# NingZhang1/pyscf_isdf

Measured on AMD Instinct MI355X. Metric: isdf_build_plus_get_jk_wall_time, lower is better.
Workload: dtype f64

## Files before the change

### include/mi355_isdf.h

```cpp
#ifndef MI355_ISDF_H
#define MI355_ISDF_H

#include <stdint.h>

#ifdef __cplusplus
extern "C" {
#endif

typedef struct isdf_ctx* isdf_handle;

#define ISDF_OK 0
#define ISDF_ERR_ARG 1
#define ISDF_ERR_HIP 2
#define ISDF_ERR_LIB 3
#define ISDF_ERR_NUM 4

int isdf_abi_version(void);

int isdf_create(int device_id, isdf_handle* out);
int isdf_destroy(isdf_handle h);
int isdf_set_stream(isdf_handle h, void* hip_stream);
const char* isdf_last_error(isdf_handle h);
int64_t isdf_workspace_bytes(isdf_handle h);
int isdf_release_workspace(isdf_handle h);
// ... 24 lines not shown
                          const double* d_coords, int64_t ngrids, double* d_re, double* d_im, int64_t ld,
                          int64_t plane_stride);

int isdf_eval_ao_k(isdf_handle h,
                   const int32_t* atm, int natm, const int32_t* bas, int nbas,
                   const double* env, int nenv,
                   const double* Ls, int nimgs, const double* rcut,
                   const double kpt[3], int periodic_part,
                   const double* d_coords, int64_t ngrids,
                   double* d_re, double* d_im, int64_t ld);

int isdf_block_row_absmax(isdf_handle h, const double* d_src, int nrow, int64_t ld, int nblk, const int64_t* d_blk_off,
                          double* d_out);
int isdf_gather_cols(isdf_handle h, const double* d_src, int nrow, int64_t ld_src,
                     const int64_t* d_idx, int64_t n, double* d_dst, int64_t ld_dst);

int isdf_partition_by_atom(isdf_handle h, const double* d_coords, int64_t ngrids, const double* atom_coords, int natm,
                           const double a[9], double tie_atol, int32_t* d_owner);

int isdf_select_ip(isdf_handle h, const double* d_ao, int nao, int64_t ld,
                   int nblk, const int64_t* blk_off, const int32_t* nip,
                   double tol, double tie_rtol,
                   double* d_L, int64_t ldL, int64_t* d_piv, int32_t* rank);

int isdf_select_ip_ws(isdf_handle h, const double* d_ao, int nao, int64_t ld,
                      int nblk, const int64_t* blk_off, const int32_t* nip,
                      double tol, double tie_rtol,
                      double* d_L, int64_t ldL, int64_t* d_piv, int32_t* rank,
                      void* d_work, int64_t work_bytes);
int64_t isdf_select_ip_work_bytes(int nao, int64_t m);

int isdf_select_ip_gram(isdf_handle h, double* d_A, int m, int64_t ldA, int nip, double tol, double tie_rtol,
                        int panel, int64_t* d_piv, int32_t* rank);

int isdf_select_ip_cplx(isdf_handle h, const double* d_ao, int nao, int nh, int64_t ld,
                        int nblk, const int64_t* blk_off, const int32_t* nip,
                        double tol, double tie_rtol,
                        double* d_L, int64_t ldL, int64_t* d_piv, int32_t* rank);

int isdf_fit_from_chol(isdf_handle h, double* d_L, int k, int64_t m, int64_t ldL,
                       const int64_t* d_piv);

int isdf_fit_prepare(isdf_handle h, const double* d_ao, int nao, int64_t ld,
                     const int64_t* d_ip, int P, double reg_rel, double* d_aoP, double* d_chol,
                     double* reg_used);
int isdf_fit_apply(isdf_handle h, const double* d_chol, const double* d_aoP, int P, int nao,
                   const double* d_ao, int64_t ng, int64_t ld, int forward_only,
                   double* d_theta, int64_t ldt);
int isdf_fit_prepare_cplx(isdf_handle h, const double* d_ao, int nao, int nh, int64_t ld,
                          const int64_t* d_ip, int P, double reg_rel, double* d_aoP, double* d_chol,
                          double* reg_used);
int isdf_fit_apply_cplx(isdf_handle h, const double* d_chol, const double* d_aoP, int P, int nao, int nh,
                        const double* d_ao, int64_t ng, int64_t ld, int forward_only,
                        double* d_theta, int64_t ldt);
int isdf_fit_global(isdf_handle h, const double* d_ao, int nao, int64_t ngrids, int64_t ld,
                    const int64_t* d_ip, int P, double reg_rel, double* d_theta, int64_t ldt,
                    double* d_aoP, double* reg_used);

int isdf_gather_aoP(isdf_handle h, const double* d_ao, int nao, int64_t ld, const int64_t* d_ip, int P,
                    double* d_aoP);
int isdf_gram_sq(isdf_handle h, const double* d_aoP, int P, int nao, int nh, double* d_A);
int isdf_pair_gram_rows(isdf_handle h, const double* d_aoP, int P, int nao, int nh, const double* d_ao,
                        int64_t ng, int64_t ld, double* d_B, int64_t ldb);
int isdf_block_chol(isdf_handle h, const double* d_A, int P, int nblk, const int32_t* blk_off,
                    double shift_rel, double* d_D, double* shift_used);
int isdf_block_solve(isdf_handle h, const double* d_D, int P, int nblk, const int32_t* blk_off, int side,
// ... 144 lines not shown
```

### pyscf_isdf_amd/backend.py

```python
import ctypes
import os
import numpy as np
import torch
from . import lib as _lib

_vp = ctypes.c_void_p


def _np_ptr(a):
    return a.ctypes.data_as(_vp)


class HipBackend:
    name = 'hip-gfx950'

    def __init__(self, device=0):
        if not torch.cuda.is_available():
            raise _lib.IsdfError('no GPU visible to torch; the ISDF path has no CPU fallback')
        self.device = torch.device('cuda', device)
        torch.cuda.set_device(self.device)
        self.handle = _lib.Handle(device)
        if os.environ.get('ISDF_TRSM') == 'subst':
            self.set_option('trsm_substitution', 1)
        if os.environ.get('ISDF_OWN_FFT') in ('0', '1', '2'):
# ... 157 lines not shown
        self._stream()
        coords_soa = self.to_device(np.ascontiguousarray(np.asarray(coords, dtype=np.float64).T))
        atoms = np.ascontiguousarray(atom_coords, dtype=np.float64)
        a = np.ascontiguousarray(a, dtype=np.float64)
        G = coords_soa.shape[1]
        owner = self.empty((G,), dtype=torch.int32)
        self.handle.call('isdf_partition_by_atom', self._p(coords_soa), G, _np_ptr(atoms), len(atoms), _np_ptr(a), float(tie_atol),
                         self._p(owner))
        return self.to_host(owner)

    def select_ip_work_bytes(self, nao, m):
        return int(self.handle.lib.isdf_select_ip_work_bytes(int(nao), int(m)))

    def select_ip(self, ao, blk_off, nip, tol, tie_rtol, L, piv, work=None):
        self._stream()
        blk_off = np.ascontiguousarray(blk_off, dtype=np.int64)
        nip = np.ascontiguousarray(nip, dtype=np.int32)
        rank = np.zeros(len(nip), dtype=np.int32)
        assert piv.dtype == torch.int64 and piv.is_contiguous() and ao.stride(1) == 1 and L.stride(1) == 1
        assert work is None or work.is_contiguous()
        self.handle.call('isdf_select_ip_ws', self._p(ao), ao.shape[0], ao.stride(0), len(nip), _np_ptr(blk_off),
                         _np_ptr(nip), float(tol), float(tie_rtol), self._p(L), L.stride(0), self._p(piv), _np_ptr(rank),
                         None if work is None else self._p(work), 0 if work is None else work.numel() * work.element_size())
        return rank

    def select_ip_gram(self, A, nip, tol, tie_rtol, piv, panel=0):
        self._stream()
        assert piv.dtype == torch.int64 and piv.is_contiguous() and A.stride(1) == 1 and A.shape[0] == A.shape[1]
        rank = ctypes.c_int32(0)
        self.handle.call('isdf_select_ip_gram', self._p(A), A.shape[0], A.stride(0), int(nip), float(tol), float(tie_rtol),
                         int(panel), self._p(piv), ctypes.byref(rank))
        return int(rank.value)

    def fit_from_chol(self, L, k, m, piv):
        self._stream()
        self.handle.call('isdf_fit_from_chol', self._p(L), int(k), int(m), L.stride(0), self._p(piv))

    def fit_prepare(self, ao, ip, reg_rel, aoP, chol):
        self._stream()
        assert ip.dtype == torch.int64 and aoP.is_contiguous() and chol.is_contiguous()
        reg = ctypes.c_double(0.0)
        self.handle.call('isdf_fit_prepare', self._p(ao), ao.shape[0], ao.stride(0), self._p(ip), ip.numel(),
                         float(reg_rel), self._p(aoP), self._p(chol), ctypes.byref(reg))
        return reg.value

    def fit_apply(self, chol, aoP, ao, ng, theta, forward_only=False):
        self._stream()
        self.handle.call('isdf_fit_apply', self._p(chol), self._p(aoP), aoP.shape[0], aoP.shape[1], self._p(ao),
                         int(ng), ao.stride(0), int(bool(forward_only)), self._p(theta), theta.stride(0))

    def gather_aoP(self, ao, ip, aoP):
        self._stream()
        self.handle.call('isdf_gather_aoP', self._p(ao), ao.shape[0], ao.stride(0), self._p(ip), ip.numel(), self._p(aoP))

    def gram_sq(self, aoP, A, nh=0):
        self._stream()
        self.handle.call('isdf_gram_sq', self._p(aoP), aoP.shape[0], aoP.shape[1], int(nh), self._p(A))

    def pair_gram_rows(self, aoP, ao, ng, B, nh=0):
        self._stream()
        self.handle.call('isdf_pair_gram_rows', self._p(aoP), aoP.shape[0], aoP.shape[1], int(nh), self._p(ao), int(ng),
                         ao.stride(0), self._p(B), B.stride(0))

    def gram_prod(self, aoP, psiP, A):
        self._stream()
        assert aoP.is_contiguous() and psiP.is_contiguous() and A.is_contiguous() and aoP.shape[0] == psiP.shape[0]
# ... 476 lines not shown
```

### pyscf_isdf_amd/csrc/common.h

```cpp
#pragma once
#include <hip/hip_runtime.h>
#include <rocblas/rocblas.h>
#include <rocsolver/rocsolver.h>
#include <hipfft/hipfft.h>
#include <cstdint>
#include <cstdio>
#include <cstring>
#include <string>
#include <vector>
#include <map>
#include "../../include/mi355_isdf.h"

struct FftPlan {
  hipfftHandle fwd = 0, bwd = 0;
  size_t work_bytes = 0;
};

struct ProfRec {
  hipEvent_t e0 = nullptr, e1 = nullptr;
};
struct ProfEntry {
  std::vector<ProfRec> recs;
  double work = 0.0;
  double ms = 0.0;
  int64_t launches = 0;
};

struct WsKernel {
  double alpha = 0.0;
  double ak[9] = {0};
  int mesh[3] = {0, 0, 0};
  double maxq[3] = {0, 0, 0};
  const double* vq = nullptr;
};

struct isdf_ctx {
  int profiling = 0;
  std::map<std::string, ProfEntry> prof;
  int device = 0;
  hipStream_t stream = nullptr;
  rocblas_handle blas = nullptr;
  std::string err;
  std::map<std::vector<int>, FftPlan> plans;
  std::map<std::string, std::pair<void*, size_t>> ws;
  int num_cu = 256;
  int trsm_substitution = 0;
  int own_fft = 2;
  int gemm_nn_own = 0;
  int attr_gemm_b = 0, attr_gemm_nn = 0, attr_gram_tri = 0, attr_herm = 0;
  int cand_gram = 1;
  int conv_pipe = 1;
  int conv_sub_rows = 0;
  int gram_pivot_tpb = 256;
  int gram_compact = 1;
  int gram_compact_permille = 875;
  int block_apply_waves = 16;
  int block_apply_reg = 1;
  double coul_omega = 0.0;
  double coul_rc = 0.0;
  int coul_sphere = 0;
  WsKernel wsk;
};

int isdf_fail(isdf_handle h, int code, const char* fmt, ...);
void* isdf_ws(isdf_handle h, const char* name, size_t bytes);
int isdf_get_plan(isdf_handle h, const int32_t mesh[3], int batch, FftPlan** out);
int get_coulG_half(isdf_handle h, const int32_t mesh[3], const double a[9], double extra_scale, double** out);
bool conv_rows_own_supported(const int32_t mesh[3], int nb);
bool conv_rows_q_own_supported(isdf_handle h, const int32_t mesh[3], int nb);
bool spectral_rows_own_supported(isdf_handle h, const int32_t mesh[3], int nb);
int spectral_rows_own(isdf_handle h, const double* d_in, int nb, const int32_t mesh[3], const int32_t* d_idx, const double* d_scale,
                      int npts, double* d_out, int64_t ldx, HIP_vector_type<double, 2u>* zbuf);
int conv_rows_q_own(isdf_handle h, const double* d_in, double* d_re, double* d_im, int nb, const int32_t mesh[3], const double* tab,
                    double2* zhalf, double2* zfull);
int conv_rows_own(isdf_handle h, const double* d_in, double* d_out, int nb, const int32_t mesh[3], const double* cg,
                  double2* zbuf);

#define HIP_TRY(h, expr)                                                                    \
  do {                                                                                      \
    hipError_t e_ = (expr);                                                                 \
    if (e_ != hipSuccess)                                                                   \
      return isdf_fail(h, ISDF_ERR_HIP, "%s:%d %s -> %s", __FILE__, __LINE__, #expr,        \
                       hipGetErrorString(e_));                                              \
  } while (0)
#define BLAS_TRY(h, expr)                                                                   \
  do {                                                                                      \
    rocblas_status s_ = (expr);                                                             \
    if (s_ != rocblas_status_success)                                                       \
// ... 35 lines not shown
  }
};

int gemm_nt_f64(isdf_handle h, int M, int N, int64_t K, double alpha, const double* A, int64_t lda,
                const double* B, int64_t ldb, double beta, double* C, int64_t ldc);
int gemm_nt_f64_scaled(isdf_handle h, int M, int N, int64_t K, double alpha, const double* A, int64_t lda,
                       const double* B, int64_t ldb, const double* kscale, double beta, double* C,
                       int64_t ldc);
int trsm_lower_left(isdf_handle h, bool trans, int m, int64_t n, const double* L, int64_t ldl, double* X, int64_t ldx);
int trsm_lower_right(isdf_handle h, bool trans, int m, int64_t n, const double* L, int64_t ldl, double* X, int64_t ldx);
int block_forward_solve(isdf_handle h, const double* D, int64_t ldd, int nblk, const int32_t* blk_off_host, double* X,
                        int64_t ldx, int64_t n);
int block_apply_inverse(isdf_handle h, const double* Dinv, int64_t ldd, int nblk, const int32_t* blk_off_host, double* X,
                        int64_t ldx, int64_t n, bool square_input = false);
int transpose_rm(isdf_handle h, const double* src, int64_t lds, int64_t rows, int64_t cols, double* dst, int64_t ldd);
int tri_left(isdf_handle h, bool trans, int m, int64_t n, const double* L, int64_t ldl, double* X, int64_t ldx);
int tri_right(isdf_handle h, bool trans, int m, int64_t n, const double* L, int64_t ldl, double* X, int64_t ldx);
bool gemm_nn_f64_supported(isdf_handle h, int64_t M, int64_t N, int64_t K, const double* A, int64_t lda, const double* B,
                           int64_t ldb);
int gemm_nn_f64(isdf_handle h, int64_t M, int64_t N, int64_t K, const double* A, int64_t lda, const double* B, int64_t ldb,
                double* C, int64_t ldc, bool square);
int gemm_rm(isdf_handle h, char opA, char opB, int64_t M, int64_t N, int64_t K, double alpha,
            const double* A, int64_t lda, const double* B, int64_t ldb, double beta, double* C,
            int64_t ldc);

__host__ __device__ inline int64_t gram_tri_row(int64_t r) {
  const int64_t tm = r >> 8;
  return 32768 * tm * (tm + 1) + (r & 255) * ((tm + 1) << 8);
}
static inline int64_t gram_tri_size(int64_t m) { return m > 0 ? gram_tri_row(m - 1) + (((m - 1) >> 8) + 1) * 256 : 0; }
struct GramTriUnit { int blk, tm, tn, pad; };
int gram_tri_blocks(isdf_handle h, const double* X, int64_t ldx, int K, const GramTriUnit* d_units, int64_t nunits,
                    const int64_t* d_blk_off, int64_t row0, const int64_t* d_tri_off, double* S, double flop);
```

### pyscf_isdf_amd/csrc/gemm_f64.hip

```cpp
#include "common.h"
#include <cstdlib>

int gemm_rm(isdf_handle h, char opA, char opB, int64_t M, int64_t N, int64_t K, double alpha,
            const double* A, int64_t lda, const double* B, int64_t ldb, double beta, double* C,
            int64_t ldc) {
  ARG_CHECK(h, M < 2147483647LL && N < 2147483647LL && K < 2147483647LL && lda < 2147483647LL &&
                   ldb < 2147483647LL && ldc < 2147483647LL);
  const rocblas_operation ta = (opA == 'N') ? rocblas_operation_none : rocblas_operation_transpose;
  const rocblas_operation tb = (opB == 'N') ? rocblas_operation_none : rocblas_operation_transpose;
  ProfScope ps(h, "rocblas_dgemm[flop]", 2.0 * M * N * (double)K);
  BLAS_TRY(h, rocblas_dgemm(h->blas, tb, ta, (rocblas_int)N, (rocblas_int)M, (rocblas_int)K, &alpha, B,
                            (rocblas_int)ldb, A, (rocblas_int)lda, &beta, C, (rocblas_int)ldc));
  return ISDF_OK;
}

namespace {

typedef double d4 __attribute__((ext_vector_type(4)));

constexpr int BM = 128, BN = 128, BK = 16;
constexpr int LDT = 17;
constexpr int TPB = 256;

struct GemmArgs {
// ... 148 lines not shown
struct GramTriArgs {
  const double* X; int64_t ldx; int K;
  const GramTriUnit* units;
  const int64_t* blk_off;
  int64_t row0;
  const int64_t* tri_off;
  double* S;
  int64_t nunits, nunits_pad;
};

__global__ __launch_bounds__(TPB2, 2) void gram_tri_mfma_kernel(GramTriArgs t) {
  extern __shared__ double smem[];
  const int64_t bid = blockIdx.x;
  const int64_t per_xcd = t.nunits_pad / 8;
  const int64_t unit = (bid % 8) * per_xcd + bid / 8;
  if (unit >= t.nunits) return;
  const GramTriUnit u = t.units[unit];
  const int64_t r0 = t.blk_off[u.blk];
  GemmArgs g;
  g.A = g.B = t.X + (r0 - t.row0) * t.ldx;
  g.lda = g.ldb = t.ldx;
  g.kscale = nullptr;
  g.M = g.N = (int)(t.blk_off[u.blk + 1] - r0);
  g.K = g.kslab = t.K;
  g.ldp = (int64_t)(u.tm + 1) * BM2;
  g.P = t.S + t.tri_off[u.blk] + (gram_tri_row((int64_t)u.tm * BM2) - (int64_t)u.tm * BM2 * g.ldp);
  g.slab_stride = 0;
  g.direct = 1; g.alpha = 1.0; g.beta = 0.0;
  constexpr bool SCALED = false;
  double* sA = smem;
  double* sB = smem + 2 * BM2 * LDT;
  const int tm = u.tm, tn = u.tn, slab = 0;
#include "gemm_nt_b_unit.inc"
}

constexpr int TPBD = 256;

template <bool SCALED>
__global__ __launch_bounds__(TPBD, 2) void gemm_nt_mfma_kernel_d(GemmArgs g) {
  __shared__ double sB[2][BN * LDT];
  const int64_t bid = blockIdx.x;
  const int64_t per_xcd = g.nunits_pad / 8;
  const int64_t unit = (bid % 8) * per_xcd + bid / 8;
  if (unit >= g.nunits) return;
  const int tm = (int)(unit % g.ntm);
  const int tn = (int)((unit / g.ntm) % g.ntn);
  const int slab = (int)(unit / ((int64_t)g.ntm * g.ntn));
  const int64_t k0 = (int64_t)slab * g.kslab;
  const int64_t k1 = (k0 + g.kslab < g.K) ? k0 + g.kslab : g.K;
  const int nchunks = (int)((k1 - k0) / BK);
  const int last = nchunks - 1;

  const int tid = threadIdx.x;
  const int lane = tid & 63, wave = tid >> 6;
  const int frow = lane & 15, fkq = lane >> 4;
  const int mlast = g.M - 1, nlast = g.N - 1;
  const double* pA0 = g.A + (int64_t)min(tm * BM + wave * 32 + frow, mlast) * g.lda + k0 + 4 * fkq;
  const double* pA1 = g.A + (int64_t)min(tm * BM + wave * 32 + 16 + frow, mlast) * g.lda + k0 + 4 * fkq;
  const int srow = tid >> 2, sseg = tid & 3;
  const double* pB0 = g.B + (int64_t)min(tn * BN + srow, nlast) * g.ldb + k0 + 4 * sseg;
  const double* pB1 = g.B + (int64_t)min(tn * BN + srow + 64, nlast) * g.ldb + k0 + 4 * sseg;
  const double* pS = SCALED ? g.kscale + k0 + 4 * sseg : nullptr;

  double2 xa00, xa01, xa10, xa11, xb00, xb01, xb10, xb11;
  double2 ya00, ya01, ya10, ya11, yb00, yb01, yb10, yb11;
#define ISDF_LOADD(C, A00, A01, A10, A11, B00, B01, B10, B11)                                 \
// ... 540 lines not shown
}

int gemm_nt_f64(isdf_handle h, int M, int N, int64_t K, double alpha, const double* A, int64_t lda,
                const double* B, int64_t ldb, double beta, double* C, int64_t ldc) {
  return gemm_nt_f64_scaled(h, M, N, K, alpha, A, lda, B, ldb, nullptr, beta, C, ldc);
}

extern "C" int isdf_gemm_nt(isdf_handle h, int M, int N, int64_t K, double alpha, const double* d_A,
                            int64_t lda, const double* d_B, int64_t ldb, const double* d_kscale,
                            double beta, double* d_C, int64_t ldc) {
  if (!h) return ISDF_ERR_ARG;
  return gemm_nt_f64_scaled(h, M, N, K, alpha, d_A, lda, d_B, ldb, d_kscale, beta, d_C, ldc);
}

int gram_tri_blocks(isdf_handle h, const double* X, int64_t ldx, int K, const GramTriUnit* d_units, int64_t nunits,
                    const int64_t* d_blk_off, int64_t row0, const int64_t* d_tri_off, double* S, double flop) {
  ARG_CHECK(h, X && d_units && d_blk_off && d_tri_off && S && nunits > 0 && K > 0 && K % 32 == 0 && ldx >= K && ldx % 2 == 0 &&
                   ((uintptr_t)X) % 16 == 0);
  GramTriArgs t;
  t.X = X; t.ldx = ldx; t.K = K; t.units = d_units; t.blk_off = d_blk_off; t.row0 = row0; t.tri_off = d_tri_off; t.S = S;
  t.nunits = nunits; t.nunits_pad = cdiv(nunits, 8) * 8;
  ARG_CHECK(h, t.nunits_pad < 2147483647LL);
  const size_t lds = sizeof(double) * 2 * (BM2 + BN) * LDT;
  if (!h->attr_gram_tri) {
    HIP_TRY(h, hipFuncSetAttribute((const void*)gram_tri_mfma_kernel, hipFuncAttributeMaxDynamicSharedMemorySize, (int)lds));
    h->attr_gram_tri = 1;
  }
  ProfScope ps(h, "cand_gram_blocks[flop]", flop);
  hipLaunchKernelGGL(gram_tri_mfma_kernel, dim3((unsigned)t.nunits_pad), dim3(TPB2), lds, h->stream, t);
  KERNEL_CHECK(h);
  return ISDF_OK;
}

bool gemm_nn_f64_supported(isdf_handle h, int64_t M, int64_t N, int64_t K, const double* A, int64_t lda, const double* B,
                           int64_t ldb) {
  return h->gemm_nn_own && M > BM && (double)(cdiv(M, BM2) * BM2) <= 1.15 * (double)M && N >= 2 && N % 2 == 0 && K >= 32 && K % 32 == 0 &&
         lda % 2 == 0 && ldb % 2 == 0 && ((uintptr_t)A) % 16 == 0 && ((uintptr_t)B) % 16 == 0 && M < 2147483647LL &&
         N < 2147483647LL && K < 2147483647LL;
}

int gemm_nn_f64(isdf_handle h, int64_t M, int64_t N, int64_t K, const double* A, int64_t lda, const double* B, int64_t ldb,
                double* C, int64_t ldc, bool square) {
  ARG_CHECK(h, A && B && C && lda >= K && ldb >= N && ldc >= N && gemm_nn_f64_supported(h, M, N, K, A, lda, B, ldb));
  GemmNNArgs g;
  g.A = A; g.lda = lda; g.B = B; g.ldb = ldb; g.C = C; g.ldc = ldc;
  g.M = (int)M; g.N = (int)N; g.K = (int)K;
  g.ntm = (int)cdiv(M, BM2); g.ntn = (int)cdiv(N, BN);
  g.stm = g.ntm >= 4 ? 4 : (g.ntm >= 2 ? 2 : 1);
  g.stn = 32 / g.stm;
  g.ngm = (int)cdiv(g.ntm, g.stm);
  g.nunits = (int64_t)g.ngm * cdiv(g.ntn, g.stn) * 32;
  g.nunits_pad = cdiv(g.nunits, 8) * 8;
  ARG_CHECK(h, g.nunits_pad < 2147483647LL);
  const size_t lds = sizeof(double) * 2 * (BM2 * LDT + BK * LDN);
  if (!h->attr_gemm_nn) {
    HIP_TRY(h, hipFuncSetAttribute((const void*)gemm_nn_mfma_kernel<true>, hipFuncAttributeMaxDynamicSharedMemorySize, (int)lds));
    HIP_TRY(h, hipFuncSetAttribute((const void*)gemm_nn_mfma_kernel<false>, hipFuncAttributeMaxDynamicSharedMemorySize, (int)lds));
    h->attr_gemm_nn = 1;
  }
  ProfScope ps(h, square ? "gemm_nn_mfma_kernel<true>[flop]" : "gemm_nn_mfma_kernel<false>[flop]", 2.0 * M * N * (double)K);
  if (square) hipLaunchKernelGGL(gemm_nn_mfma_kernel<true>, dim3((unsigned)g.nunits_pad), dim3(TPB2), lds, h->stream, g);
  else hipLaunchKernelGGL(gemm_nn_mfma_kernel<false>, dim3((unsigned)g.nunits_pad), dim3(TPB2), lds, h->stream, g);
  KERNEL_CHECK(h);
  return ISDF_OK;
}
```

### pyscf_isdf_amd/csrc/gemm_nt_b_unit.inc

```
  const int64_t k0 = (int64_t)slab * g.kslab;
  const int64_t k1 = (k0 + g.kslab < g.K) ? k0 + g.kslab : g.K;
  const int nchunks = (int)((k1 - k0) / BK);
  const int last = nchunks - 1;

  const int tid = threadIdx.x;
  const int lane = tid & 63, wave = tid >> 6;
  const int wm = wave >> 1, wn = wave & 1;
  const int srow = tid >> 3;
  const int sseg = tid & 7;
  const int mlast = g.M - 1, nlast = g.N - 1;
  const double* pA0 = g.A + (int64_t)min(tm * BM2 + srow, mlast) * g.lda + k0 + sseg * 2;
  const double* pA1 = g.A + (int64_t)min(tm * BM2 + srow + 64, mlast) * g.lda + k0 + sseg * 2;
  const double* pA2 = g.A + (int64_t)min(tm * BM2 + srow + 128, mlast) * g.lda + k0 + sseg * 2;
  const double* pA3 = g.A + (int64_t)min(tm * BM2 + srow + 192, mlast) * g.lda + k0 + sseg * 2;
  const double* pB0 = g.B + (int64_t)min(tn * BN + srow, nlast) * g.ldb + k0 + sseg * 2;
  const double* pB1 = g.B + (int64_t)min(tn * BN + srow + 64, nlast) * g.ldb + k0 + sseg * 2;
  const double* pS = SCALED ? g.kscale + k0 + sseg * 2 : nullptr;

  double2 xa0, xa1, xa2, xa3, xb0, xb1, ya0, ya1, ya2, ya3, yb0, yb1;
#define ISDF_LOADB(C, A0, A1, A2, A3, B0, B1)                                                 \
  {                                                                                           \
    const int off = (C) * BK;                                                                 \
    A0 = *reinterpret_cast<const double2*>(pA0 + off);                                        \
    A1 = *reinterpret_cast<const double2*>(pA1 + off);                                        \
// ... 56 lines not shown
  {                                                                                           \
    ISDF_FRAGQ(BUF, 1, a1, b1)                                                                \
    LOAD_AHEAD                                                                                \
    ISDF_MFMAB(a0, b0)                                                                        \
    ISDF_INTERLEAVE_L()                                                                       \
    __builtin_amdgcn_sched_barrier(0);                                                        \
    ISDF_FRAGQ(BUF, 2, a0, b0)                                                                \
    ISDF_MFMAB(a1, b1)                                                                        \
    ISDF_INTERLEAVE()                                                                         \
    __builtin_amdgcn_sched_barrier(0);                                                        \
    ISDF_FRAGQ(BUF, 3, a1, b1)                                                                \
    STORE_NEXT                                                                                \
    ISDF_MFMAB(a0, b0)                                                                        \
    ISDF_INTERLEAVE_RW()                                                                      \
    __builtin_amdgcn_sched_barrier(0);                                                        \
    __syncthreads();                                                                          \
    ISDF_FRAGQ(1 - (BUF), 0, a0, b0)                                                          \
    ISDF_MFMAB(a1, b1)                                                                        \
    ISDF_INTERLEAVE()                                                                         \
    __builtin_amdgcn_sched_barrier(0);                                                        \
  }

  ISDF_LOADB(0, xa0, xa1, xa2, xa3, xb0, xb1)
  ISDF_LOADB(1, ya0, ya1, ya2, ya3, yb0, yb1)
  ISDF_STOREB(0, xa0, xa1, xa2, xa3, xb0, xb1)
  __syncthreads();
  ISDF_FRAGQ(0, 0, a0, b0)
  __builtin_amdgcn_sched_barrier(0);
  for (int c = 0; c < nchunks; c += 2) {
    ISDF_CHUNKB(0, ISDF_LOADB(min(c + 2, last), xa0, xa1, xa2, xa3, xb0, xb1), ISDF_STOREB(1, ya0, ya1, ya2, ya3, yb0, yb1))
    ISDF_CHUNKB(1, ISDF_LOADB(min(c + 3, last), ya0, ya1, ya2, ya3, yb0, yb1), ISDF_STOREB(0, xa0, xa1, xa2, xa3, xb0, xb1))
  }

  double* out = g.P + (int64_t)slab * g.slab_stride;
#pragma unroll
  for (int i = 0; i < 4; ++i) {
#pragma unroll
    for (int r = 0; r < 4; ++r) {
      const int row = tm * BM2 + wm * 64 + i * 16 + (lane >> 4) + 4 * r;
      if (row >= g.M) continue;
#pragma unroll
      for (int j = 0; j < 4; ++j) {
        const int col = tn * BN + wn * 64 + j * 16 + (lane & 15);
        if (col >= g.N) continue;
        double* q = out + (int64_t)row * g.ldp + col;
        const double v = acc[i][j][r];
        if (g.direct) *q = (g.beta == 0.0) ? g.alpha * v : g.alpha * v + g.beta * (*q);
        else *q = v;
      }
    }
  }
```

### pyscf_isdf_amd/csrc/handle.hip

```cpp
#include "common.h"
#include <cstdarg>

int isdf_fail(isdf_handle h, int code, const char* fmt, ...) {
  char buf[1024];
  va_list ap;
  va_start(ap, fmt);
  vsnprintf(buf, sizeof(buf), fmt, ap);
  va_end(ap);
  if (h) h->err = buf;
  else fprintf(stderr, "mi355_isdf: %s\n", buf);
  return code;
}

void* isdf_ws(isdf_handle h, const char* name, size_t bytes) {
  auto& slot = h->ws[name];
  if (slot.second >= bytes && slot.first) return slot.first;
  if (slot.first) {
    (void)hipStreamSynchronize(h->stream);
    (void)hipFree(slot.first);
    slot.first = nullptr;
    slot.second = 0;
  }
  void* p = nullptr;
  hipError_t e = hipMalloc(&p, bytes ? bytes : 8);
// ... 49 lines not shown
  ARG_CHECK(h, rc >= 0.0);
  h->coul_rc = rc;
  return ISDF_OK;
}

int isdf_set_coulomb_ws(isdf_handle h, double alpha, const double ak[9], const int32_t mesh[3], const double maxq[3],
                        const double* d_vq) {
  if (!h) return ISDF_ERR_ARG;
  if (alpha <= 0.0) { h->wsk = WsKernel(); return ISDF_OK; }
  ARG_CHECK(h, ak && mesh && maxq && d_vq && mesh[0] > 0 && mesh[1] > 0 && mesh[2] > 0);
  h->wsk.alpha = alpha;
  for (int i = 0; i < 9; ++i) h->wsk.ak[i] = ak[i];
  for (int i = 0; i < 3; ++i) { h->wsk.mesh[i] = mesh[i]; h->wsk.maxq[i] = maxq[i]; }
  h->wsk.vq = d_vq;
  return ISDF_OK;
}

int isdf_set_option(isdf_handle h, const char* key, int value) {
  if (!h) return ISDF_ERR_ARG;
  ARG_CHECK(h, key != nullptr);
  if (std::string(key) == "trsm_substitution") { h->trsm_substitution = value ? 1 : 0; return ISDF_OK; }
  if (std::string(key) == "own_fft") { h->own_fft = value < 0 ? 0 : (value > 2 ? 2 : value); return ISDF_OK; }
  if (std::string(key) == "gemm_nn_own") { h->gemm_nn_own = value ? 1 : 0; return ISDF_OK; }
  if (std::string(key) == "coul_sphere") { h->coul_sphere = value < 0 ? 0 : value; return ISDF_OK; }
  if (std::string(key) == "conv_pipe") { h->conv_pipe = value != 0; return ISDF_OK; }
  if (std::string(key) == "conv_sub_rows") { h->conv_sub_rows = value < 0 ? 0 : value; return ISDF_OK; }
  if (std::string(key) == "gram_pivot_tpb") {
    if (value != 64 && value != 128 && value != 256) return ISDF_ERR_ARG;
    h->gram_pivot_tpb = value;
    return ISDF_OK;
  }
  if (std::string(key) == "cand_gram") { h->cand_gram = value ? 1 : 0; return ISDF_OK; }
  if (std::string(key) == "gram_compact") { h->gram_compact = value ? 1 : 0; return ISDF_OK; }
  if (std::string(key) == "gram_compact_permille") {
    if (value < 1 || value > 1000) return isdf_fail(h, ISDF_ERR_ARG, "isdf_set_option: gram_compact_permille %d not in [1, 1000]", value);
    h->gram_compact_permille = value;
    return ISDF_OK;
  }
  if (std::string(key) == "block_apply_waves") { h->block_apply_waves = value < 1 ? 1 : value; return ISDF_OK; }
  if (std::string(key) == "block_apply_reg") { h->block_apply_reg = value ? 1 : 0; return ISDF_OK; }
  return isdf_fail(h, ISDF_ERR_ARG, "isdf_set_option: unknown key '%s'", key);
}

int isdf_create(int device_id, isdf_handle* out) {
  if (!out) return ISDF_ERR_ARG;
  *out = nullptr;
  int ndev = 0;
  hipError_t e = hipGetDeviceCount(&ndev);
  if (e != hipSuccess || ndev == 0)
    return isdf_fail(nullptr, ISDF_ERR_HIP, "no HIP device visible (%s)", hipGetErrorString(e));
  if (device_id < 0 || device_id >= ndev)
    return isdf_fail(nullptr, ISDF_ERR_ARG, "device %d out of range (%d devices)", device_id, ndev);
  isdf_ctx* h = new isdf_ctx();
  h->device = device_id;
  if (hipSetDevice(device_id) != hipSuccess) { delete h; return ISDF_ERR_HIP; }
  hipDeviceProp_t prop;
  if (hipGetDeviceProperties(&prop, device_id) == hipSuccess) h->num_cu = prop.multiProcessorCount;
  if (rocblas_create_handle(&h->blas) != rocblas_status_success) {
    delete h;
    return isdf_fail(nullptr, ISDF_ERR_LIB, "rocblas_create_handle failed");
  }
  rocblas_set_pointer_mode(h->blas, rocblas_pointer_mode_host);
  *out = h;
  return ISDF_OK;
}

// ... 80 lines not shown
```

### pyscf_isdf_amd/csrc/select_gram.hip

```cpp
#include "common.h"
#include <cfloat>
#include <climits>

namespace {

constexpr int PANEL_MAX = 256;
constexpr int SW = 2048;

struct GramState {
  double tol;
  int rank;
  int done;
};

__device__ inline double wmax(double v) {
  for (int o = 32; o > 0; o >>= 1) v = fmax(v, __shfl_xor(v, o));
  return v;
}
__device__ inline int wmin(int v) {
  for (int o = 32; o > 0; o >>= 1) {
    int u = __shfl_xor(v, o);
    v = u < v ? u : v;
  }
  return v;
// ... 172 lines not shown
    wgmax[blockIdx.x] = mx;
  }
}

__global__ __launch_bounds__(256) void gram_piv_to_original_kernel(int64_t* __restrict__ piv, int j0, int j1,
                                                                   const int32_t* __restrict__ cmap) {
  const int j = j0 + blockIdx.x * 256 + threadIdx.x;
  if (j < j1) piv[j] = cmap[piv[j]];
}

__global__ __launch_bounds__(256) void gram_compact_gather_kernel(const double* __restrict__ A, int64_t ldA,
                                                                  const int32_t* __restrict__ map, int mc, int r0,
                                                                  double* __restrict__ S, int64_t lds) {
  const int r = r0 + blockIdx.y;
  const int i = blockIdx.x * 256 + threadIdx.x;
  const int ncol = min(mc, (r / SW + 1) * SW);
  if (i >= ncol) return;
  const int mr = map[r], mi = map[i];
  S[(int64_t)blockIdx.y * lds + i] = (mr >= (mi / SW) * SW) ? A[(int64_t)mr * ldA + mi] : A[(int64_t)mi * ldA + mr];
}

__global__ __launch_bounds__(256) void gram_compact_store_kernel(const double* __restrict__ S, int64_t lds, int mc, int r0,
                                                                 double* __restrict__ A, int64_t ldA) {
  const int r = r0 + blockIdx.y;
  const int i = blockIdx.x * 256 + threadIdx.x;
  const int ncol = min(mc, (r / SW + 1) * SW);
  if (i >= ncol) return;
  A[(int64_t)r * ldA + i] = S[(int64_t)blockIdx.y * lds + i];
}

}

namespace {
struct DeviceBuffer {
  void* p = nullptr;
  ~DeviceBuffer() { if (p) (void)hipFree(p); }
};
constexpr int COMPACT_ROWS = 512;
}

extern "C" int isdf_select_ip_gram(isdf_handle h, double* d_A, int m, int64_t ldA, int nip, double tol,
                                   double tie_rtol, int panel, int64_t* d_piv, int32_t* rank) {
  if (!h) return ISDF_ERR_ARG;
  ARG_CHECK(h, d_A && d_piv && rank);
  ARG_CHECK(h, m > 0 && ldA >= m && nip > 0 && tie_rtol >= 0.0 && tie_rtol < 1.0);
  if (panel <= 0) panel = 256;
  ARG_CHECK(h, panel <= PANEL_MAX);
  if (nip > m) nip = m;
  const int TPB = h->gram_pivot_tpb;
  int nwg = (int)cdiv(m, TPB);
  const int64_t ldL = ((int64_t)m + 31) / 32 * 32;
  auto al = [](size_t x) { return (x + 255) / 256 * 256; };
  const size_t b_d = al(sizeof(double) * m), b_w = al(sizeof(double) * nwg), b_st = al(sizeof(GramState));
  const size_t b_L = al(sizeof(double) * (size_t)panel * ldL), b_map = al(sizeof(int32_t) * m);
  char* ws = (char*)isdf_ws(h, "select_gram", 2 * b_d + 2 * b_w + b_st + b_L + 3 * b_map);
  if (!ws) return ISDF_ERR_HIP;
  double* d_d[2];
  double* d_w[2];
  d_d[0] = (double*)ws; ws += b_d;
  d_d[1] = (double*)ws; ws += b_d;
  d_w[0] = (double*)ws; ws += b_w;
  d_w[1] = (double*)ws; ws += b_w;
  GramState* d_st = (GramState*)ws; ws += b_st;
  double* d_Lp = (double*)ws; ws += b_L;
  int32_t* d_map = (int32_t*)ws; ws += b_map;
  int32_t* d_cmap[2];
  d_cmap[0] = (int32_t*)ws; ws += b_map;
  d_cmap[1] = (int32_t*)ws;
  HIP_TRY(h, hipMemsetAsync(d_st, 0, sizeof(GramState), h->stream));
  HIP_TRY(h, hipMemsetAsync(d_piv, 0xff, sizeof(int64_t) * (size_t)nip, h->stream));
  if (TPB == 64) hipLaunchKernelGGL(gram_diag_kernel<64>, dim3(nwg), dim3(64), 0, h->stream, d_A, ldA, m, d_d[0], d_w[0]);
  else if (TPB == 128) hipLaunchKernelGGL(gram_diag_kernel<128>, dim3(nwg), dim3(128), 0, h->stream, d_A, ldA, m, d_d[0], d_w[0]);
  else hipLaunchKernelGGL(gram_diag_kernel<256>, dim3(nwg), dim3(256), 0, h->stream, d_A, ldA, m, d_d[0], d_w[0]);
  KERNEL_CHECK(h);
  int ms = m;
  int rank_at_compact = 0;
  int cc = -1;
  auto piv_to_original = [&](int j1) -> int {
    if (cc < 0 || j1 <= rank_at_compact) return ISDF_OK;
    hipLaunchKernelGGL(gram_piv_to_original_kernel, dim3((unsigned)cdiv(j1 - rank_at_compact, 256)), dim3(256), 0, h->stream,
                       d_piv, rank_at_compact, j1, (const int32_t*)d_cmap[cc]);
    KERNEL_CHECK(h);
    return ISDF_OK;
  };
  std::vector<int32_t> cmap_h, map_h;
  std::vector<double> d_h;
  bool compact = h->gram_compact != 0;
  DeviceBuffer stage;
  int64_t stage_ld = 0;
  int cur = 0;
  for (int k0 = 0; k0 < nip; k0 += panel) {
    const int nb = nip - k0 < panel ? nip - k0 : panel;
    {
      ProfScope ps(h, "gram_pivot_step_kernel[byte]", 8.0 * (double)ms * (0.5 * nb * (nb - 1) + 4.0 * nb), nb);
      for (int jl = 0; jl < nb; ++jl) {
#define ISDF_GRAM_STEP(T)                                                                                              \
  hipLaunchKernelGGL(gram_pivot_step_kernel<T>, dim3(nwg), dim3(T), 0, h->stream, d_A, ldA, ms, d_Lp, ldL, d_d[cur],    \
                     d_d[cur ^ 1], d_w[cur], d_w[cur ^ 1], nwg, k0 + jl, jl, nip, tol, tie_rtol, d_st, d_piv)
        if (TPB == 64) ISDF_GRAM_STEP(64);
        else if (TPB == 128) ISDF_GRAM_STEP(128);
        else ISDF_GRAM_STEP(256);
#undef ISDF_GRAM_STEP
        cur ^= 1;
      }
      KERNEL_CHECK(h);
    }
    GramState hst;
    HIP_TRY(h, hipMemcpyAsync(&hst, d_st, sizeof(GramState), hipMemcpyDeviceToHost, h->stream));
    HIP_TRY(h, hipStreamSynchronize(h->stream));
    if (k0 + nb >= nip) break;
    int mc = ms;
    if (compact && !hst.done && ((int64_t)ms - (hst.rank - rank_at_compact)) * 1000 < (int64_t)ms * h->gram_compact_permille) {
      d_h.resize(ms);
      HIP_TRY(h, hipMemcpyAsync(d_h.data(), d_d[cur], sizeof(double) * ms, hipMemcpyDeviceToHost, h->stream));
      HIP_TRY(h, hipStreamSynchronize(h->stream));
      map_h.clear();
      for (int i = 0; i < ms; ++i)
        if (!(d_h[i] < 0.0)) map_h.push_back(i);
      mc = (int)map_h.size();
      if (mc > 0 && mc < ms && !stage.p) {
        stage_ld = ((int64_t)mc + 31) / 32 * 32;
        if (hipMalloc(&stage.p, sizeof(double) * (size_t)COMPACT_ROWS * stage_ld) != hipSuccess) {
          (void)hipGetLastError();
          stage.p = nullptr;
          fprintf(stderr, "mi355_isdf: isdf_select_ip_gram: no device memory for the compaction's staging rows (%zu bytes); "
                          "the pick goes on over the whole matrix\n", sizeof(double) * (size_t)COMPACT_ROWS * stage_ld);
          compact = false;
          mc = ms;
        }
      }
    }
    for (int c0 = 0; c0 < ms; c0 += SW) {
      const int c1 = c0 + SW < ms ? c0 + SW : ms;
      int rc = gemm_rm(h, 'T', 'N', ms - c0, c1 - c0, nb, -1.0, d_Lp + c0, ldL, d_Lp + c0, ldL, 1.0,
                       d_A + (int64_t)c0 * ldA + c0, ldA);
      if (rc != ISDF_OK) return rc;
    }
    if (mc == 0 || mc == ms) continue;
    std::vector<int32_t> cm(mc);
    for (int i = 0; i < mc; ++i) cm[i] = cmap_h.empty() ? map_h[i] : cmap_h[map_h[i]];
    cmap_h.swap(cm);
    int rc = piv_to_original(hst.rank);
    if (rc) return rc;
    cc = cc < 0 ? 0 : cc ^ 1;
    HIP_TRY(h, hipMemcpyAsync(d_map, map_h.data(), sizeof(int32_t) * mc, hipMemcpyHostToDevice, h->stream));
    HIP_TRY(h, hipMemcpyAsync(d_cmap[cc], cmap_h.data(), sizeof(int32_t) * mc, hipMemcpyHostToDevice, h->stream));
    {
      ProfScope ps(h, "gram_compact[byte]", 32.0 * 0.5 * (double)mc * mc, 1);
      const int nwc = (int)cdiv(mc, TPB);
      if (TPB == 64) hipLaunchKernelGGL(gram_compact_diag_kernel<64>, dim3(nwc), dim3(64), 0, h->stream, d_d[cur], d_map, mc, d_d[cur ^ 1], d_w[cur ^ 1]);
      else if (TPB == 128) hipLaunchKernelGGL(gram_compact_diag_kernel<128>, dim3(nwc), dim3(128), 0, h->stream, d_d[cur], d_map, mc, d_d[cur ^ 1], d_w[cur ^ 1]);
      else hipLaunchKernelGGL(gram_compact_diag_kernel<256>, dim3(nwc), dim3(256), 0, h->stream, d_d[cur], d_map, mc, d_d[cur ^ 1], d_w[cur ^ 1]);
      KERNEL_CHECK(h);
      for (int r0 = 0; r0 < mc; r0 += COMPACT_ROWS) {
        const int nr = mc - r0 < COMPACT_ROWS ? mc - r0 : COMPACT_ROWS;
        const int ncol = (r0 / SW + 1) * SW < mc ? (r0 / SW + 1) * SW : mc;
        const dim3 grid((unsigned)cdiv(ncol, 256), (unsigned)nr);
        hipLaunchKernelGGL(gram_compact_gather_kernel, grid, dim3(256), 0, h->stream, d_A, ldA, d_map, mc, r0,
                           (double*)stage.p, stage_ld);
        hipLaunchKernelGGL(gram_compact_store_kernel, grid, dim3(256), 0, h->stream, (const double*)stage.p, stage_ld, mc,
                           r0, d_A, ldA);
      }
      KERNEL_CHECK(h);
    }
    cur ^= 1;
    ms = mc;
    nwg = (int)cdiv(ms, TPB);
    rank_at_compact = hst.rank;
  }
  GramState hst;
  HIP_TRY(h, hipMemcpyAsync(&hst, d_st, sizeof(GramState), hipMemcpyDeviceToHost, h->stream));
  HIP_TRY(h, hipStreamSynchronize(h->stream));
  int rc = piv_to_original(hst.rank);
  if (rc) return rc;
  HIP_TRY(h, hipStreamSynchronize(h->stream));
  *rank = hst.rank;
  return ISDF_OK;
}
```

### pyscf_isdf_amd/lib.py

```python
import ctypes
import os

_HERE = os.path.dirname(os.path.abspath(__file__))
LIB_PATH = os.path.join(_HERE, 'lib', 'libmi355_isdf.so')
ABI_VERSION = 21

_lib = None

c_int, c_i64, c_dbl, c_vp = ctypes.c_int, ctypes.c_int64, ctypes.c_double, ctypes.c_void_p

SIGNATURES = {
    'isdf_abi_version': (c_int, []),
    'isdf_create': (c_int, [c_int, ctypes.POINTER(c_vp)]),
    'isdf_destroy': (c_int, [c_vp]),
    'isdf_set_stream': (c_int, [c_vp, c_vp]),
    'isdf_last_error': (ctypes.c_char_p, [c_vp]),
    'isdf_workspace_bytes': (c_i64, [c_vp]),
    'isdf_set_coulomb_omega': (c_int, [c_vp, c_dbl]),
    'isdf_set_coulomb_cutoff': (c_int, [c_vp, c_dbl]),
    'isdf_set_coulomb_ws': (c_int, [c_vp, c_dbl, c_vp, c_vp, c_vp, c_vp]),
    'isdf_set_option': (c_int, [c_vp, ctypes.c_char_p, c_int]),
    'isdf_release_workspace': (c_int, [c_vp]),
    'isdf_prof_enable': (c_int, [c_vp, c_int]),
    'isdf_prof_reset': (c_int, [c_vp]),
    'isdf_prof_count': (c_int, [c_vp]),
    'isdf_prof_get': (c_int, [c_vp, c_int, ctypes.c_char_p, c_int, ctypes.POINTER(c_i64), ctypes.POINTER(c_dbl), ctypes.POINTER(c_dbl)]),
    'isdf_eval_ao': (c_int, [c_vp, c_vp, c_int, c_vp, c_int, c_vp, c_int, c_vp, c_int, c_vp, c_vp, c_i64, c_vp, c_i64]),
    'isdf_block_row_absmax': (c_int, [c_vp, c_vp, c_int, c_i64, c_int, c_vp, c_vp]),
    'isdf_gather_cols': (c_int, [c_vp, c_vp, c_int, c_i64, c_vp, c_i64, c_vp, c_i64]),
    'isdf_partition_by_atom': (c_int, [c_vp, c_vp, c_i64, c_vp, c_int, c_vp, c_dbl, c_vp]),
    'isdf_select_ip': (c_int, [c_vp, c_vp, c_int, c_i64, c_int, c_vp, c_vp, c_dbl, c_dbl, c_vp, c_i64, c_vp, c_vp]),
    'isdf_select_ip_ws': (c_int, [c_vp, c_vp, c_int, c_i64, c_int, c_vp, c_vp, c_dbl, c_dbl, c_vp, c_i64, c_vp, c_vp, c_vp,
                                  c_i64]),
    'isdf_select_ip_work_bytes': (c_i64, [c_int, c_i64]),
    'isdf_select_ip_gram': (c_int, [c_vp, c_vp, c_int, c_i64, c_int, c_dbl, c_dbl, c_int, c_vp, ctypes.POINTER(ctypes.c_int32)]),
    'isdf_fit_from_chol': (c_int, [c_vp, c_vp, c_int, c_i64, c_i64, c_vp]),
    'isdf_fit_prepare': (c_int, [c_vp, c_vp, c_int, c_i64, c_vp, c_int, c_dbl, c_vp, c_vp, ctypes.POINTER(c_dbl)]),
    'isdf_fit_apply': (c_int, [c_vp, c_vp, c_vp, c_int, c_int, c_vp, c_i64, c_i64, c_int, c_vp, c_i64]),
    'isdf_gather_aoP': (c_int, [c_vp, c_vp, c_int, c_i64, c_vp, c_int, c_vp]),
    'isdf_gram_sq': (c_int, [c_vp, c_vp, c_int, c_int, c_int, c_vp]),
    'isdf_pair_gram_rows': (c_int, [c_vp, c_vp, c_int, c_int, c_int, c_vp, c_i64, c_i64, c_vp, c_i64]),
    'isdf_gram_prod': (c_int, [c_vp, c_vp, c_int, c_int, c_vp, c_int, c_vp]),
    'isdf_pair_prod_rows': (c_int, [c_vp, c_vp, c_int, c_int, c_vp, c_int, c_vp, c_i64, c_vp, c_i64, c_i64, c_vp, c_i64]),
    'isdf_factor_solve_half': (c_int, [c_vp, c_vp, c_int, c_int, c_vp, c_i64, c_i64]),
    'isdf_gram_prod_cplx': (c_int, [c_vp, c_vp, c_int, c_int, c_int, c_vp, c_int, c_int, c_vp]),
    'isdf_pair_prod_rows_cplx': (c_int, [c_vp, c_vp, c_int, c_int, c_int, c_vp, c_int, c_int, c_vp, c_i64, c_vp, c_i64, c_i64,
                                         c_vp, c_i64]),
    'isdf_block_chol': (c_int, [c_vp, c_vp, c_int, c_int, c_vp, c_dbl, c_vp, ctypes.POINTER(c_dbl)]),
    'isdf_block_solve': (c_int, [c_vp, c_vp, c_int, c_int, c_vp, c_int, c_int, c_vp, c_i64, c_i64]),
    'isdf_block_invert': (c_int, [c_vp, c_vp, c_int, c_int, c_vp, c_vp]),
    'isdf_block_apply': (c_int, [c_vp, c_vp, c_i64, c_int, c_vp, c_vp, c_i64, c_i64]),
    'isdf_pair_rows_block_apply': (c_int, [c_vp, c_vp, c_int, c_int, c_vp, c_i64, c_i64, c_vp, c_i64, c_int, c_vp, c_vp, c_i64]),
    'isdf_shift_diag': (c_int, [c_vp, c_vp, c_int, c_dbl]),
    'isdf_chol_inplace': (c_int, [c_vp, c_vp, c_int, c_dbl, c_vp, ctypes.POINTER(c_dbl)]),
    'isdf_factor_solve': (c_int, [c_vp, c_vp, c_int, c_vp, c_i64, c_i64]),
    'isdf_bj_probe_vectors': (c_int, [c_vp, c_vp, c_int, c_vp, c_vp, c_int, c_int, c_vp]),
    'isdf_rows_combine': (c_int, [c_vp, c_vp, c_int, c_i64, c_int, c_vp, c_i64, c_i64, c_vp, c_i64, c_int]),
    'isdf_bj_probe_rows': (c_int, [c_vp, c_vp, c_int, c_vp, c_vp, c_int, c_int, c_vp, c_vp, c_i64, c_i64, c_vp, c_i64]),
    'isdf_gather_T': (c_int, [c_vp, c_vp, c_int, c_i64, c_vp, c_vp]),
    'isdf_W_from_factor': (c_int, [c_vp, c_vp, c_int, c_int, c_vp, c_i64]),
    'isdf_fit_global': (c_int, [c_vp, c_vp, c_int, c_i64, c_i64, c_vp, c_int, c_dbl, c_vp, c_i64, c_vp, ctypes.POINTER(c_dbl)]),
    'isdf_coulomb_W': (c_int, [c_vp, c_vp, c_int, c_i64, c_vp, c_vp, c_int, c_int, c_int, c_int, c_vp, c_i64]),
    'isdf_coulomb_rows': (c_int, [c_vp, c_vp, c_int, c_i64, c_vp, c_vp, c_int, c_vp, c_i64]),
    'isdf_symmetrize_upper': (c_int, [c_vp, c_vp, c_int, c_i64]),
    'isdf_symmetrize_mean': (c_int, [c_vp, c_vp, c_int, c_i64, c_int]),
    'isdf_get_j': (c_int, [c_vp, c_vp, c_int, c_i64, c_i64, c_vp, c_vp, c_vp, c_int, c_vp]),
    'isdf_rho': (c_int, [c_vp, c_vp, c_int, c_i64, c_i64, c_vp, c_int, c_vp, c_i64]),
    'isdf_coulomb_potential': (c_int, [c_vp, c_vp, c_int, c_i64, c_vp, c_vp]),
# ... 104 lines not shown
```

Baseline: 17.02.

## Replace strip-wise rocBLAS trailing Gram update with one fused MFMA kernel launch

```diff
diff --git a/include/mi355_isdf.h b/include/mi355_isdf.h
--- a/include/mi355_isdf.h
+++ b/include/mi355_isdf.h
@@ -80,6 +80,8 @@
 
 int isdf_select_ip_gram(isdf_handle h, double* d_A, int m, int64_t ldA, int nip, double tol, double tie_rtol,
                         int panel, int64_t* d_piv, int32_t* rank);
+
+int isdf_gram_trailing_update(isdf_handle h, double* d_A, int ms, int64_t ldA, const double* d_Lp, int64_t ldL, int nb);
 
 int isdf_select_ip_cplx(isdf_handle h, const double* d_ao, int nao, int nh, int64_t ld,
                         int nblk, const int64_t* blk_off, const int32_t* nip,
diff --git a/pyscf_isdf_amd/backend.py b/pyscf_isdf_amd/backend.py
--- a/pyscf_isdf_amd/backend.py
+++ b/pyscf_isdf_amd/backend.py
@@ -213,6 +213,12 @@
                          int(panel), self._p(piv), ctypes.byref(rank))
         return int(rank.value)
 
+    def gram_trailing_update(self, A, Lp):
+        self._stream()
+        assert A.stride(1) == 1 and Lp.stride(1) == 1 and A.shape[0] == A.shape[1] == Lp.shape[1]
+        self.handle.call('isdf_gram_trailing_update', self._p(A), A.shape[0], A.stride(0), self._p(Lp), Lp.stride(0),
+                         Lp.shape[0])
+
     def fit_from_chol(self, L, k, m, piv):
         self._stream()
         self.handle.call('isdf_fit_from_chol', self._p(L), int(k), int(m), L.stride(0), self._p(piv))
diff --git a/pyscf_isdf_amd/csrc/common.h b/pyscf_isdf_amd/csrc/common.h
--- a/pyscf_isdf_amd/csrc/common.h
+++ b/pyscf_isdf_amd/csrc/common.h
@@ -47,13 +47,14 @@
   int trsm_substitution = 0;
   int own_fft = 2;
   int gemm_nn_own = 0;
-  int attr_gemm_b = 0, attr_gemm_nn = 0, attr_gram_tri = 0, attr_herm = 0;
+  int attr_gemm_b = 0, attr_gemm_nn = 0, attr_gram_tri = 0, attr_herm = 0, attr_gram_update = 0;
   int cand_gram = 1;
   int conv_pipe = 1;
   int conv_sub_rows = 0;
   int gram_pivot_tpb = 256;
   int gram_compact = 1;
   int gram_compact_permille = 875;
+  int gram_update_own = 1;
   int block_apply_waves = 16;
   int block_apply_reg = 1;
   double coul_omega = 0.0;
@@ -155,3 +156,7 @@
 struct GramTriUnit { int blk, tm, tn, pad; };
 int gram_tri_blocks(isdf_handle h, const double* X, int64_t ldx, int K, const GramTriUnit* d_units, int64_t nunits,
                     const int64_t* d_blk_off, int64_t row0, const int64_t* d_tri_off, double* S, double flop);
+
+struct GramUpdateUnit { int tm, tn; };
+int gram_update_blocks(isdf_handle h, const double* T, int64_t ldt, int K, const GramUpdateUnit* d_units, int64_t nunits,
+                       double* A, int64_t ldA, int ms);
diff --git a/pyscf_isdf_amd/csrc/gemm_f64.hip b/pyscf_isdf_amd/csrc/gemm_f64.hip
--- a/pyscf_isdf_amd/csrc/gemm_f64.hip
+++ b/pyscf_isdf_amd/csrc/gemm_f64.hip
@@ -204,6 +204,38 @@
   double* sB = smem + 2 * BM2 * LDT;
   const int tm = u.tm, tn = u.tn, slab = 0;
 #include "gemm_nt_b_unit.inc"
+}
+
+struct GramUpdateArgs {
+  const double* T; int64_t ldt; int K;
+  const GramUpdateUnit* units;
+  double* A; int64_t ldA; int ms;
+  int64_t nunits, nunits_pad;
+};
+
+__global__ __launch_bounds__(TPB2, 2) void gram_update_mfma_kernel(GramUpdateArgs t) {
+  extern __shared__ double smem[];
+  const int64_t bid = blockIdx.x;
+  const int64_t per_xcd = t.nunits_pad / 8;
+  const int64_t unit = (bid % 8) * per_xcd + bid / 8;
+  if (unit >= t.nunits) return;
+  const GramUpdateUnit u = t.units[unit];
+  GemmArgs g;
+  g.A = g.B = t.T;
+  g.lda = g.ldb = t.ldt;
+  g.kscale = nullptr;
+  g.M = g.N = t.ms;
+  g.K = g.kslab = t.K;
+  g.P = t.A; g.ldp = t.ldA;
+  g.slab_stride = 0;
+  g.direct = 1; g.alpha = -1.0; g.beta = 1.0;
+  constexpr bool SCALED = false;
+  double* sA = smem;
+  double* sB = smem + 2 * BM2 * LDT;
+  const int tm = u.tm, tn = u.tn, slab = 0;
+#define ISDF_UNIT_RMW_EPILOGUE
+#include "gemm_nt_b_unit.inc"
+#undef ISDF_UNIT_RMW_EPILOGUE
 }
 
 constexpr int TPBD = 256;
@@ -810,6 +842,24 @@
   return ISDF_OK;
 }
 
+int gram_update_blocks(isdf_handle h, const double* T, int64_t ldt, int K, const GramUpdateUnit* d_units, int64_t nunits,
+                       double* A, int64_t ldA, int ms) {
+  ARG_CHECK(h, T && d_units && A && nunits > 0 && ms > 0 && ldA >= ms && K > 0 && K % 32 == 0 && ldt >= K && ldt % 2 == 0 &&
+                   ((uintptr_t)T) % 16 == 0);
+  GramUpdateArgs t;
+  t.T = T; t.ldt = ldt; t.K = K; t.units = d_units; t.A = A; t.ldA = ldA; t.ms = ms;
+  t.nunits = nunits; t.nunits_pad = cdiv(nunits, 8) * 8;
+  ARG_CHECK(h, t.nunits_pad < 2147483647LL);
+  const size_t lds = sizeof(double) * 2 * (BM2 + BN) * LDT;
+  if (!h->attr_gram_update) {
+    HIP_TRY(h, hipFuncSetAttribute((const void*)gram_update_mfma_kernel, hipFuncAttributeMaxDynamicSharedMemorySize, (int)lds));
+    h->attr_gram_update = 1;
+  }
+  hipLaunchKernelGGL(gram_update_mfma_kernel, dim3((unsigned)t.nunits_pad), dim3(TPB2), lds, h->stream, t);
+  KERNEL_CHECK(h);
+  return ISDF_OK;
+}
+
 bool gemm_nn_f64_supported(isdf_handle h, int64_t M, int64_t N, int64_t K, const double* A, int64_t lda, const double* B,
                            int64_t ldb) {
   return h->gemm_nn_own && M > BM && (double)(cdiv(M, BM2) * BM2) <= 1.15 * (double)M && N >= 2 && N % 2 == 0 && K >= 32 && K % 32 == 0 &&
diff --git a/pyscf_isdf_amd/csrc/gemm_nt_b_unit.inc b/pyscf_isdf_amd/csrc/gemm_nt_b_unit.inc
--- a/pyscf_isdf_amd/csrc/gemm_nt_b_unit.inc
+++ b/pyscf_isdf_amd/csrc/gemm_nt_b_unit.inc
@@ -112,6 +112,38 @@
     ISDF_CHUNKB(1, ISDF_LOADB(min(c + 3, last), ya0, ya1, ya2, ya3, yb0, yb1), ISDF_STOREB(0, xa0, xa1, xa2, xa3, xb0, xb1))
   }
 
+#ifdef ISDF_UNIT_RMW_EPILOGUE
+  {
+    double* out = g.P;
+    const int col0 = tn * BN + wn * 64 + (lane & 15);
+#pragma unroll
+    for (int ih = 0; ih < 4; ih += 2) {
+      double cv[2][4][4];
+#pragma unroll
+      for (int i = 0; i < 2; ++i)
+#pragma unroll
+        for (int r = 0; r < 4; ++r) {
+          const int row = tm * BM2 + wm * 64 + (ih + i) * 16 + (lane >> 4) + 4 * r;
+#pragma unroll
+          for (int j = 0; j < 4; ++j) {
+            const int col = col0 + j * 16;
+            cv[i][r][j] = (row < g.M && col < g.N) ? __builtin_nontemporal_load(out + (int64_t)row * g.ldp + col) : 0.0;
+          }
+        }
+#pragma unroll
+      for (int i = 0; i < 2; ++i)
+#pragma unroll
+        for (int r = 0; r < 4; ++r) {
+          const int row = tm * BM2 + wm * 64 + (ih + i) * 16 + (lane >> 4) + 4 * r;
+#pragma unroll
+          for (int j = 0; j < 4; ++j) {
+            const int col = col0 + j * 16;
+            if (row < g.M && col < g.N) __builtin_nontemporal_store(cv[i][r][j] - acc[ih + i][j][r], out + (int64_t)row * g.ldp + col);
+          }
+        }
+    }
+  }
+#else
   double* out = g.P + (int64_t)slab * g.slab_stride;
 #pragma unroll
   for (int i = 0; i < 4; ++i) {
@@ -130,3 +162,4 @@
       }
     }
   }
+#endif
diff --git a/pyscf_isdf_amd/csrc/handle.hip b/pyscf_isdf_amd/csrc/handle.hip
--- a/pyscf_isdf_amd/csrc/handle.hip
+++ b/pyscf_isdf_amd/csrc/handle.hip
@@ -105,6 +105,7 @@
   }
   if (std::string(key) == "cand_gram") { h->cand_gram = value ? 1 : 0; return ISDF_OK; }
   if (std::string(key) == "gram_compact") { h->gram_compact = value ? 1 : 0; return ISDF_OK; }
+  if (std::string(key) == "gram_update_own") { h->gram_update_own = value ? 1 : 0; return ISDF_OK; }
   if (std::string(key) == "gram_compact_permille") {
     if (value < 1 || value > 1000) return isdf_fail(h, ISDF_ERR_ARG, "isdf_set_option: gram_compact_permille %d not in [1, 1000]", value);
     h->gram_compact_permille = value;
diff --git a/pyscf_isdf_amd/csrc/select_gram.hip b/pyscf_isdf_amd/csrc/select_gram.hip
--- a/pyscf_isdf_amd/csrc/select_gram.hip
+++ b/pyscf_isdf_amd/csrc/select_gram.hip
@@ -228,6 +228,66 @@
 }
 
 namespace {
+void gram_update_units(int ms, std::vector<GramUpdateUnit>& units, double* entries) {
+  constexpr int PR = 4, PC = 8, TS_M = SW / 256, TS_N = SW / 128;
+  const int ntm = (int)cdiv(ms, 256), ntn = (int)cdiv(ms, 128);
+  units.clear();
+  double e = 0.0;
+  for (int s = 0; s * TS_N < ntn; ++s) {
+    const int tn1 = (s + 1) * TS_N < ntn ? (s + 1) * TS_N : ntn;
+    for (int rg = s * TS_M; rg < ntm; rg += PR)
+      for (int cg = s * TS_N; cg < tn1; cg += PC)
+        for (int tn = cg; tn < cg + PC && tn < tn1; ++tn)
+          for (int tm = rg; tm < rg + PR && tm < ntm; ++tm) {
+            units.push_back(GramUpdateUnit{tm, tn});
+            e += (double)((tm + 1) * 256 < ms ? 256 : ms - tm * 256) * (double)((tn + 1) * 128 < ms ? 128 : ms - tn * 128);
+          }
+  }
+  *entries = e;
+}
+
+int gram_update_strips(isdf_handle h, double* d_A, int ms, int64_t ldA, const double* d_Lp, int64_t ldL, int nb) {
+  for (int c0 = 0; c0 < ms; c0 += SW) {
+    const int c1 = c0 + SW < ms ? c0 + SW : ms;
+    int rc = gemm_rm(h, 'T', 'N', ms - c0, c1 - c0, nb, -1.0, d_Lp + c0, ldL, d_Lp + c0, ldL, 1.0,
+                     d_A + (int64_t)c0 * ldA + c0, ldA);
+    if (rc != ISDF_OK) return rc;
+  }
+  return ISDF_OK;
+}
+
+int gram_update_own(isdf_handle h, double* d_A, int ms, int64_t ldA, const double* d_Lp, int64_t ldL, int nb, double* d_T,
+                    const GramUpdateUnit* d_units, int64_t nunits, double entries) {
+  const int K32 = (nb + 31) / 32 * 32;
+  ProfScope ps(h, "gram_trailing_update[flop]", 2.0 * nb * entries);
+  if (K32 != nb) HIP_TRY(h, hipMemsetAsync(d_T, 0, sizeof(double) * (size_t)ms * K32, h->stream));
+  int rc = transpose_rm(h, d_Lp, ldL, nb, ms, d_T, K32);
+  if (rc != ISDF_OK) return rc;
+  return gram_update_blocks(h, d_T, K32, K32, d_units, nunits, d_A, ldA, ms);
+}
+}
+
+extern "C" int isdf_gram_trailing_update(isdf_handle h, double* d_A, int ms, int64_t ldA, const double* d_Lp, int64_t ldL,
+                                         int nb) {
+  if (!h) return ISDF_ERR_ARG;
+  ARG_CHECK(h, d_A && d_Lp && ms > 0 && ldA >= ms && ldL >= ms && nb > 0);
+  const int K32 = (nb + 31) / 32 * 32;
+  if (!h->gram_update_own || K32 > PANEL_MAX) return gram_update_strips(h, d_A, ms, ldA, d_Lp, ldL, nb);
+  std::vector<GramUpdateUnit> units;
+  double entries = 0.0;
+  gram_update_units(ms, units, &entries);
+  const size_t b_T = (sizeof(double) * (size_t)ms * K32 + 255) / 256 * 256;
+  char* ws = (char*)isdf_ws(h, "gram_update", b_T + sizeof(GramUpdateUnit) * units.size());
+  if (!ws) return ISDF_ERR_HIP;
+  GramUpdateUnit* d_units = (GramUpdateUnit*)(ws + b_T);
+  HIP_TRY(h, hipMemcpyAsync(d_units, units.data(), sizeof(GramUpdateUnit) * units.size(), hipMemcpyHostToDevice, h->stream));
+  int rc = gram_update_own(h, d_A, ms, ldA, d_Lp, ldL, nb, (double*)ws, d_units, (int64_t)units.size(), entries);
+  if (rc != ISDF_OK) return rc;
+  HIP_TRY(h, hipStreamSynchronize(h->stream));
+  return ISDF_OK;
+}
+
+namespace {
 struct DeviceBuffer {
   void* p = nullptr;
   ~DeviceBuffer() { if (p) (void)hipFree(p); }
@@ -249,7 +309,20 @@
   auto al = [](size_t x) { return (x + 255) / 256 * 256; };
   const size_t b_d = al(sizeof(double) * m), b_w = al(sizeof(double) * nwg), b_st = al(sizeof(GramState));
   const size_t b_L = al(sizeof(double) * (size_t)panel * ldL), b_map = al(sizeof(int32_t) * m);
-  char* ws = (char*)isdf_ws(h, "select_gram", 2 * b_d + 2 * b_w + b_st + b_L + 3 * b_map);
+  const int K32max = (panel + 31) / 32 * 32;
+  bool own = h->gram_update_own != 0 && K32max <= PANEL_MAX;
+  std::vector<GramUpdateUnit> units_h;
+  double upd_entries = 0.0;
+  if (own) gram_update_units(m, units_h, &upd_entries);
+  const size_t b_T = al(sizeof(double) * (size_t)m * K32max), b_un = al(sizeof(GramUpdateUnit) * units_h.size());
+  const size_t b_base = 2 * b_d + 2 * b_w + b_st + b_L + 3 * b_map;
+  char* ws = own ? (char*)isdf_ws(h, "select_gram", b_base + b_T + b_un) : nullptr;
+  if (own && !ws) {
+    fprintf(stderr, "mi355_isdf: isdf_select_ip_gram: no device memory for the transposed panel of the trailing update (%zu bytes); "
+                    "the updates go through rocBLAS\n", b_T + b_un);
+    own = false;
+  }
+  if (!ws) ws = (char*)isdf_ws(h, "select_gram", b_base);
   if (!ws) return ISDF_ERR_HIP;
   double* d_d[2];
   double* d_w[2];
@@ -262,7 +335,10 @@
   int32_t* d_map = (int32_t*)ws; ws += b_map;
   int32_t* d_cmap[2];
   d_cmap[0] = (int32_t*)ws; ws += b_map;
-  d_cmap[1] = (int32_t*)ws;
+  d_cmap[1] = (int32_t*)ws; ws += b_map;
+  double* d_T = (double*)ws; ws += b_T;
+  GramUpdateUnit* d_units = (GramUpdateUnit*)ws;
+  if (own) HIP_TRY(h, hipMemcpyAsync(d_units, units_h.data(), sizeof(GramUpdateUnit) * units_h.size(), hipMemcpyHostToDevice, h->stream));
   HIP_TRY(h, hipMemsetAsync(d_st, 0, sizeof(GramState), h->stream));
   HIP_TRY(h, hipMemsetAsync(d_piv, 0xff, sizeof(int64_t) * (size_t)nip, h->stream));
   if (TPB == 64) hipLaunchKernelGGL(gram_diag_kernel<64>, dim3(nwg), dim3(64), 0, h->stream, d_A, ldA, m, d_d[0], d_w[0]);
@@ -326,10 +402,9 @@
         }
       }
     }
-    for (int c0 = 0; c0 < ms; c0 += SW) {
-      const int c1 = c0 + SW < ms ? c0 + SW : ms;
-      int rc = gemm_rm(h, 'T', 'N', ms - c0, c1 - c0, nb, -1.0, d_Lp + c0, ldL, d_Lp + c0, ldL, 1.0,
-                       d_A + (int64_t)c0 * ldA + c0, ldA);
+    {
+      const int rc = own ? gram_update_own(h, d_A, ms, ldA, d_Lp, ldL, nb, d_T, d_units, (int64_t)units_h.size(), upd_entries)
+                         : gram_update_strips(h, d_A, ms, ldA, d_Lp, ldL, nb);
       if (rc != ISDF_OK) return rc;
     }
     if (mc == 0 || mc == ms) continue;
@@ -362,6 +437,10 @@
     cur ^= 1;
     ms = mc;
     nwg = (int)cdiv(ms, TPB);
+    if (own) {
+      gram_update_units(ms, units_h, &upd_entries);
+      HIP_TRY(h, hipMemcpyAsync(d_units, units_h.data(), sizeof(GramUpdateUnit) * units_h.size(), hipMemcpyHostToDevice, h->stream));
+    }
     rank_at_compact = hst.rank;
   }
   GramState hst;
diff --git a/pyscf_isdf_amd/lib.py b/pyscf_isdf_amd/lib.py
--- a/pyscf_isdf_amd/lib.py
+++ b/pyscf_isdf_amd/lib.py
@@ -34,6 +34,7 @@
                                   c_i64]),
     'isdf_select_ip_work_bytes': (c_i64, [c_int, c_i64]),
     'isdf_select_ip_gram': (c_int, [c_vp, c_vp, c_int, c_i64, c_int, c_dbl, c_dbl, c_int, c_vp, ctypes.POINTER(ctypes.c_int32)]),
+    'isdf_gram_trailing_update': (c_int, [c_vp, c_vp, c_int, c_i64, c_vp, c_i64, c_int]),
     'isdf_fit_from_chol': (c_int, [c_vp, c_vp, c_int, c_i64, c_i64, c_vp]),
     'isdf_fit_prepare': (c_int, [c_vp, c_vp, c_int, c_i64, c_vp, c_int, c_dbl, c_vp, c_vp, ctypes.POINTER(c_dbl)]),
     'isdf_fit_apply': (c_int, [c_vp, c_vp, c_vp, c_int, c_int, c_vp, c_i64, c_i64, c_int, c_vp, c_i64]),
```

New measurement: 16.89, median of 6. Within noise of the previous version (-0.8%).
